# zju3dv/Diffuman4D

Hardware: NVIDIA H100
Metric: unet_window_denoise_steps_per_sec (higher is better)
Workload: dtype bf16

## Files before the change

diffuman4d_b200/csrc/common.cuh:

```cuda
#pragma once
#include <cuda.h>
#include <cuda_bf16.h>
#include <cuda_runtime.h>
#include <stdint.h>
#include <string>

namespace d4d {

typedef __nv_bfloat16 bf16;

void set_error(const std::string& msg);
#define D4D_CUDA_OK(expr)                                                                        \
  do {                                                                                           \
    cudaError_t _e = (expr);                                                                     \
    if (_e != cudaSuccess) {                                                                     \
      d4d::set_error(std::string(#expr) + " failed: " + cudaGetErrorString(_e) + " @" + __FILE__ + \
                     ":" + std::to_string(__LINE__));                                            \
      return 2;                                                                                  \
    }                                                                                            \
  } while (0)
#define D4D_REQUIRE(cond, msg)                                                                   \
  do {                                                                                           \
    if (!(cond)) {                                                                               \
      d4d::set_error(std::string("invalid argument: ") + msg + " (" #cond ") @" + __FILE__ + ":" + \
                     std::to_string(__LINE__));                                                  \
      return 1;                                                                                  \
    }                                                                                            \
  } while (0)

int make_tmap_2d(CUtensorMap* out, const void* base, uint64_t rows, uint64_t cols, uint64_t ld,
                 uint32_t box_cols, uint32_t box_rows, int swizzle_bytes);
int make_tmap_nhwc(CUtensorMap* out, const void* base, uint64_t n, uint64_t h, uint64_t w, uint64_t c,
                   uint32_t box_c, uint32_t box_w, uint32_t box_h, uint32_t box_n, int swizzle_bytes, int stride = 1);

#ifdef __CUDACC__
__device__ __forceinline__ uint32_t smem_u32(const void* p) {
  return static_cast<uint32_t>(__cvta_generic_to_shared(p));
}
__device__ __forceinline__ bool elect_one() {
  uint32_t pred = 0;
  asm volatile(
      "{\n\t.reg .b32 rx;\n\t.reg .pred px;\n\t"
      "elect.sync rx|px, 0xffffffff;\n\t"
      "selp.b32 %0, 1, 0, px;\n\t}\n"
      : "=r"(pred));
  return pred != 0;
}

__device__ __forceinline__ void mbar_init(uint64_t* bar, uint32_t count) {
  asm volatile("mbarrier.init.shared::cta.b64 [%0], %1;" ::"r"(smem_u32(bar)), "r"(count) : "memory");
}
__device__ __forceinline__ void fence_mbar_init() {
  asm volatile("fence.mbarrier_init.release.cluster;" ::: "memory");
}
__device__ __forceinline__ void mbar_expect_tx(uint64_t* bar, uint32_t bytes) {
  asm volatile("mbarrier.arrive.expect_tx.shared::cta.b64 _, [%0], %1;" ::"r"(smem_u32(bar)), "r"(bytes)
               : "memory");
}
__device__ __forceinline__ void mbar_arrive(uint64_t* bar) {
  asm volatile("mbarrier.arrive.shared::cta.b64 _, [%0];" ::"r"(smem_u32(bar)) : "memory");
}
__device__ __forceinline__ bool mbar_try_wait(uint64_t* bar, uint32_t parity) {
  uint32_t ok;
  asm volatile(
      "{\n\t.reg .pred p;\n\t"
      "mbarrier.try_wait.parity.shared::cta.b64 p, [%1], %2;\n\t"
      "selp.b32 %0, 1, 0, p;\n\t}\n"
      : "=r"(ok)
      : "r"(smem_u32(bar)), "r"(parity)
      : "memory");
  return ok != 0;
}
#ifndef D4D_SPIN_LIMIT
#define D4D_SPIN_LIMIT (1u << 26)
#endif
__device__ __forceinline__ void mbar_wait(uint64_t* bar, uint32_t parity) {
  uint32_t spins = 0;
  while (!mbar_try_wait(bar, parity)) {
    if (++spins > D4D_SPIN_LIMIT) {
      printf("d4d: mbarrier timeout block=(%d,%d) thread=%d bar=%u parity=%u\n", blockIdx.x, blockIdx.y,
             threadIdx.x, smem_u32(bar), parity);
      __trap();
    }
  }
}
__device__ __forceinline__ void mbar_wait_nocall(uint64_t* bar, uint32_t parity) {
  uint32_t spins = 0;
  while (!mbar_try_wait(bar, parity)) {
    if (++spins > D4D_SPIN_LIMIT) __trap();
  }
}

__device__ __forceinline__ void fence_proxy_async_smem() {
  asm volatile("fence.proxy.async.shared::cta;" ::: "memory");
}
__device__ __forceinline__ void named_barrier_sync(int id, int threads) {
  asm volatile("bar.sync %0, %1;" ::"r"(id), "r"(threads) : "memory");
}
__device__ __forceinline__ void named_barrier_arrive(int id, int threads) {
  asm volatile("bar.arrive %0, %1;" ::"r"(id), "r"(threads) : "memory");
}
__device__ __forceinline__ void st_shared_u32(uint32_t addr, uint32_t v) {
  asm volatile("st.shared.b32 [%0], %1;" ::"r"(addr), "r"(v) : "memory");
}
__device__ __forceinline__ uint32_t ld_shared_u32(uint32_t addr) {
  uint32_t v;
  asm volatile("ld.shared.b32 %0, [%1];" : "=r"(v) : "r"(addr) : "memory");
  return v;
}
__device__ __forceinline__ void pdl_wait() { asm volatile("griddepcontrol.wait;" ::: "memory"); }
__device__ __forceinline__ void pdl_launch_dependents() { asm volatile("griddepcontrol.launch_dependents;" ::: "memory"); }
template <int R> __device__ __forceinline__ void setmaxnreg_dec() { asm volatile("setmaxnreg.dec.sync.aligned.u32 %0;" ::"n"(R)); }
template <int R> __device__ __forceinline__ void setmaxnreg_inc() { asm volatile("setmaxnreg.inc.sync.aligned.u32 %0;" ::"n"(R)); }

__device__ __forceinline__ void tma_prefetch_desc(const CUtensorMap* t) {
  asm volatile("prefetch.tensormap [%0];" ::"l"(reinterpret_cast<uint64_t>(t)) : "memory");
}
__device__ __forceinline__ void tma_load_2d(void* dst, const CUtensorMap* t, uint64_t* bar, int c0, int c1) {
  asm volatile(
      "cp.async.bulk.tensor.2d.shared::cluster.global.tile.mbarrier::complete_tx::bytes [%0], [%1, {%3, %4}], [%2];"
      ::"r"(smem_u32(dst)), "l"(reinterpret_cast<uint64_t>(t)), "r"(smem_u32(bar)), "r"(c0), "r"(c1)
      : "memory");
}
__device__ __forceinline__ void tma_load_4d(void* dst, const CUtensorMap* t, uint64_t* bar, int c0, int c1, int c2,
                                            int c3) {
  asm volatile(
      "cp.async.bulk.tensor.4d.shared::cluster.global.tile.mbarrier::complete_tx::bytes [%0], [%1, {%3, %4, %5, %6}], [%2];"
      ::"r"(smem_u32(dst)), "l"(reinterpret_cast<uint64_t>(t)), "r"(smem_u32(bar)), "r"(c0), "r"(c1), "r"(c2),
      "r"(c3)
      : "memory");
}

__device__ __forceinline__ void tma_store_2d(const CUtensorMap* t, const void* src, int c0, int c1) {
  asm volatile("cp.async.bulk.tensor.2d.global.shared::cta.bulk_group [%0, {%2, %3}], [%1];"
               ::"l"(reinterpret_cast<uint64_t>(t)), "r"(smem_u32(src)), "r"(c0), "r"(c1) : "memory");
}
__device__ __forceinline__ void bulk_commit_group() { asm volatile("cp.async.bulk.commit_group;" ::: "memory"); }
template <int N> __device__ __forceinline__ void bulk_wait_group_read() {
  asm volatile("cp.async.bulk.wait_group.read %0;" ::"n"(N) : "memory");
}
template <int N> __device__ __forceinline__ void bulk_wait_group() {
  asm volatile("cp.async.bulk.wait_group %0;" ::"n"(N) : "memory");
}

__device__ __forceinline__ uint32_t pack_bf16x2(float lo, float hi) {
  __nv_bfloat162 v = __floats2bfloat162_rn(lo, hi);
  return *reinterpret_cast<uint32_t*>(&v);
}
__device__ __forceinline__ float2 unpack_bf16x2(uint32_t u) {
  __nv_bfloat162 v = *reinterpret_cast<__nv_bfloat162*>(&u);
  return __bfloat1622float2(v);
}
__device__ __forceinline__ float silu_f(float x) { return __fdividef(x, 1.0f + __expf(-x)); }
__device__ __forceinline__ float gelu_erf_f(float g) {
  const float u = fabsf(g);
  float q = fmaf(-4.8811754095e-04f, u, 7.1988063864e-03f);
  q = fmaf(q, u, -5.2146803588e-02f);
  q = fmaf(q, u, -4.5959571004e-01f);
  q = fmaf(q, u, -1.1510006189e+00f);
  float e;
  asm("ex2.approx.ftz.f32 %0, %1;" : "=f"(e) : "f"(q * u));
  return fmaf(-0.5f * u, e, fmaxf(g, 0.f));
}
#endif

}
```

diffuman4d_b200/csrc/gemm_wgmma.cu:

```cuda
#include "kernels.h"
#include "wgmma.cuh"

namespace d4d {

namespace {

constexpr int BLOCK_M = 128;
constexpr int BLOCK_K = 64;
constexpr int A_BYTES = BLOCK_M * BLOCK_K * 2;
constexpr int BAR_BYTES = 1024;
constexpr int NUM_THREADS = 384;
constexpr int MAX_SMEM = 227 * 1024;

constexpr int SLAB_COLS = 32;
constexpr int SLAB_BYTES = 64 * SLAB_COLS * 2;

template <int BN, int MI, bool kStaged, bool kPingPong>
struct GemmCfg {
  static constexpr int TILE_A_BYTES = kPingPong ? A_BYTES : MI * A_BYTES;
  static constexpr int STAGE_BYTES = TILE_A_BYTES + BN * BLOCK_K * 2;
  static constexpr int STAGING_BYTES = kStaged ? 2 * 64 * MI * BN * 2 : 0;
  static constexpr int STAGES_FIT = (MAX_SMEM - 1024 - BAR_BYTES - STAGING_BYTES) / STAGE_BYTES;
  static constexpr int STAGES = STAGES_FIT > 8 ? 8 : STAGES_FIT;
  static constexpr int SMEM = 1024 + BAR_BYTES + STAGES * STAGE_BYTES + STAGING_BYTES;
};

struct TileCoord {
  int m0;
  int n_img0, y0, x0;
  int pa, pb;
};

template <bool kConv>
__device__ __forceinline__ void tile_coords(const GemmKernelArgs& a, int m_tile, TileCoord& t) {
  if (!kConv) {
    t.m0 = m_tile * BLOCK_M;
    t.n_img0 = t.y0 = t.x0 = 0;
    t.pa = t.pb = 0;
  } else {
    const int ph = a.n_phases > 1 ? m_tile / a.tiles_per_phase : 0;
    m_tile -= ph * a.tiles_per_phase;
    t.pa = ph >> 1;
    t.pb = ph & 1;
    int tx = m_tile % a.tiles_x;
    int r = m_tile / a.tiles_x;
    int ty = r % a.tiles_y;
    int tn = r / a.tiles_y;
    t.m0 = 0;
    t.x0 = tx * a.BW;
    t.y0 = ty * a.BH;
    t.n_img0 = tn * a.BN;
  }
}

template <bool kConv>
__device__ __forceinline__ void row_of(const GemmKernelArgs& a, const TileCoord& tc, int rr, long long& row, int& img,
                                       bool& valid) {
  if (!kConv) {
    row = static_cast<long long>(tc.m0) + rr;
    valid = row < a.M;
    img = a.rows_per_image > 0 ? static_cast<int>(row / a.rows_per_image) : 0;
  } else {
    const int bx = rr % a.BW;
    const int r2 = rr / a.BW;
    const int by = r2 % a.BH;
    const int bn = r2 / a.BH;
    const int x = tc.x0 + bx, y = tc.y0 + by, n = tc.n_img0 + bn;
    valid = (x < a.W) && (y < a.H) && (n < a.n_img);
    row = (static_cast<long long>(n) * a.out_H + (y * a.out_sy + a.out_oy + tc.pa)) * a.out_W + (x * a.out_sx + a.out_ox + tc.pb);
    img = n;
  }
}

enum : int { E_BIAS = 1, E_ROWVEC = 2, E_ACT = 4, E_RES = 8, E_STATS = 16, E_KV = 32, E_ALL = 63, E_STAGED_ALL = E_ALL & ~E_KV };
__host__ __device__ constexpr bool gemm_staged(bool conv, int epi) { return !conv && !(epi & E_KV); }

constexpr int ORDER_BAR = 3;

template <int BN, int MI, bool kGeglu, bool kConv, int kEpi, bool kPingPong>
__global__ void __launch_bounds__(NUM_THREADS, 1)
gemm_wgmma_kernel(const __grid_constant__ CUtensorMap tmap_a, const __grid_constant__ CUtensorMap tmap_a2,
                  const __grid_constant__ CUtensorMap tmap_b, const __grid_constant__ CUtensorMap tmap_c,
                  const __grid_constant__ CUtensorMap tmap_r, const GemmKernelArgs a) {
  constexpr bool kStaged = gemm_staged(kConv, kEpi);
  static_assert(MI == 1 || (kConv && MI == 2) || kPingPong, "256-row tiles: conv mode only (a plain tile is 128 rows)");
  static_assert(!kPingPong || (kStaged && MI == 2), "ping-pong: staged plain GEMMs, one warpgroup per 128-row tile");
  using Cfg = GemmCfg<BN, MI, kStaged, kPingPong>;
  constexpr int STAGES = Cfg::STAGES;
  extern __shared__ uint8_t smem_raw[];
  uint8_t* smem = reinterpret_cast<uint8_t*>((reinterpret_cast<uintptr_t>(smem_raw) + 1023) & ~uintptr_t(1023));
  uint64_t* full = reinterpret_cast<uint64_t*>(smem);
  uint64_t* empty = full + STAGES;
  uint64_t* res_full = empty + STAGES;
  uint8_t* ring = smem + BAR_BYTES;

  const int warp = __shfl_sync(0xffffffffu, threadIdx.x >> 5, 0);
  const int lane = threadIdx.x & 31;
  const int total_tiles = a.m_tiles * a.n_tiles;

  if (threadIdx.x == 0) {
    tma_prefetch_desc(&tmap_a);
    tma_prefetch_desc(&tmap_b);
    if (a.kb_split < a.k_blocks) tma_prefetch_desc(&tmap_a2);
    for (int i = 0; i < STAGES; ++i) {
      mbar_init(&full[i], 1);
      mbar_init(&empty[i], kPingPong ? 1 : 2);
    }
    mbar_init(&res_full[0], 1);
    mbar_init(&res_full[1], 1);
    fence_mbar_init();
  }
  __syncthreads();
  pdl_wait();
  pdl_launch_dependents();

  if (warp < 4) {
    setmaxnreg_dec<40>();
    if (threadIdx.x == 0) {
      const uint32_t tx_bytes = Cfg::TILE_A_BYTES + static_cast<uint32_t>(a.block_n) * BLOCK_K * 2;
      int stage = 0;
      uint32_t phase = 0;
      for (int tile = blockIdx.x; tile < total_tiles; tile += gridDim.x) {
        const int m_tile = tile / a.n_tiles;
        const int n_tile = tile % a.n_tiles;
        TileCoord tc;
        tile_coords<kConv>(a, m_tile, tc);
        const int n0 = n_tile * a.block_n;
        for (int kb = 0; kb < a.k_blocks; ++kb) {
          mbar_wait_nocall(&empty[stage], phase ^ 1);
          uint8_t* sa = ring + stage * Cfg::STAGE_BYTES;
          uint8_t* sb = sa + Cfg::TILE_A_BYTES;
          mbar_expect_tx(&full[stage], tx_bytes);
          if (!kConv) {
            if (kb < a.kb_split) tma_load_2d(sa, &tmap_a, &full[stage], kb * BLOCK_K, tc.m0);
            else tma_load_2d(sa, &tmap_a2, &full[stage], (kb - a.kb_split) * BLOCK_K, tc.m0);
            tma_load_2d(sb, &tmap_b, &full[stage], kb * BLOCK_K, n0);
          } else {
            const int tap = kb / a.cin_blocks;
            const int cb = kb - tap * a.cin_blocks;
            tma_load_4d(sa, &tmap_a, &full[stage], cb * BLOCK_K, tc.x0 * a.in_stride + a.tap_dx[tap] + tc.pb,
                        tc.y0 * a.in_stride + a.tap_dy[tap] + tc.pa, tc.n_img0);
            tma_load_2d(sb, &tmap_b, &full[stage], tap * a.Cin + cb * BLOCK_K, n0 + (tc.pa * 2 + tc.pb) * a.N);
          }
          if (++stage == STAGES) { stage = 0; phase ^= 1; }
        }
      }
    }
    return;
  }

  setmaxnreg_inc<232>();
  const int wg = (warp >> 2) - 1;
  const int wq = warp & 3;
  const bool wg_leader = (threadIdx.x & 127) == 0;
  const int wg_row0 = kPingPong ? 0 : wg * 64 * MI;
  const int r_base = wg_row0 + wq * 16 + (lane >> 2);
  const int c_base = 2 * (lane & 3);
  const uint32_t ring_u32 = smem_u32(ring);
  constexpr int STG_BLOCK = 64 * BN * 2;
  const bool staged = kStaged && a.staged;
  uint8_t* stg = ring + STAGES * Cfg::STAGE_BYTES + wg * MI * STG_BLOCK;
  const uint32_t stg_u32 = smem_u32(stg) + (r_base - wg_row0) * 64 + c_base * 2;
  const int stg_xor = (lane >> 3) & 3;
  const bool has_res = (kEpi & E_RES) && !kGeglu && a.residual != nullptr;
  const int out_cols = kGeglu ? a.N / 2 : a.N;
  uint32_t res_phase = 0;

  int stage = 0;
  uint32_t phase = 0;
  const auto skip_stages = [&](int n) {
    stage += n;
    while (stage >= STAGES) { stage -= STAGES; phase ^= 1; }
  };
  if (kPingPong && wg == 1) {
    skip_stages(a.k_blocks);
    named_barrier_arrive(ORDER_BAR, 256);
  }
  const int tile_step = kPingPong ? 2 * gridDim.x : gridDim.x;
  float acc[MI][BN / 2];
  for (int tile = blockIdx.x + (kPingPong ? wg * gridDim.x : 0); tile < total_tiles; tile += tile_step) {
    const int m_tile = tile / a.n_tiles;
    const int n_tile = tile % a.n_tiles;
    TileCoord tc;
    tile_coords<kConv>(a, m_tile, tc);
    const int n0 = n_tile * a.block_n;
    const int ocol0 = kGeglu ? n0 / 2 : n0;
    const int ocols = min(kGeglu ? a.block_n / 2 : a.block_n, out_cols - ocol0);
    const int n_slabs = (ocols + SLAB_COLS - 1) / SLAB_COLS;
    const int orow0 = tc.m0 + wg_row0;
    const int live_blocks = staged ? max(0, min(MI, (a.M - orow0 + 63) / 64)) : 0;

    if (kPingPong) named_barrier_sync(ORDER_BAR + wg, 256);
    int prev_stage = -1;
    for (int kb = 0; kb < a.k_blocks; ++kb) {
      mbar_wait_nocall(&full[stage], phase);
      const uint32_t sa = ring_u32 + stage * Cfg::STAGE_BYTES + wg_row0 * 128;
      const uint32_t sb = ring_u32 + stage * Cfg::STAGE_BYTES + Cfg::TILE_A_BYTES;
      const uint64_t adesc = make_wgmma_desc(sa, 16, 1024);
      const uint64_t bdesc = make_wgmma_desc(sb, 16, 1024);
      wgmma_fence();
#pragma unroll
      for (int k = 0; k < BLOCK_K / 16; ++k) {
        const int scale_d = (kb | k) != 0 ? 1 : 0;
#pragma unroll
        for (int mi = 0; mi < MI; ++mi) {
          const uint64_t ad = adesc + 512 * mi + 2 * k, bd = bdesc + 2 * k;
          if constexpr (BN == 64) wgmma_ss_n64(acc[mi], ad, bd, scale_d);
          else if constexpr (BN == 128) wgmma_ss_n128(acc[mi], ad, bd, scale_d);
          else if constexpr (BN == 160) wgmma_ss_n160(acc[mi], ad, bd, scale_d);
          else if constexpr (BN == 192) wgmma_ss_n192(acc[mi], ad, bd, scale_d);
          else wgmma_ss_n256(acc[mi], ad, bd, scale_d);
        }
      }
      wgmma_commit();
      if (kb == 0 && staged && wg_leader) {
        bulk_wait_group_read<0>();
        if (has_res && live_blocks > 0) {
          mbar_expect_tx(&res_full[wg], live_blocks * n_slabs * SLAB_BYTES);
          for (int mi = 0; mi < live_blocks; ++mi)
            for (int s = 0; s < n_slabs; ++s)
              tma_load_2d(stg + mi * STG_BLOCK + s * SLAB_BYTES, &tmap_r, &res_full[wg], ocol0 + s * SLAB_COLS, orow0 + 64 * mi);
        }
      }
      wgmma_wait<1>();
      if (prev_stage >= 0 && wg_leader) mbar_arrive(&empty[prev_stage]);
      prev_stage = stage;
      if (++stage == STAGES) { stage = 0; phase ^= 1; }
    }
    if (kPingPong) {
      if (tile + gridDim.x < total_tiles) named_barrier_arrive(ORDER_BAR + (wg ^ 1), 256);
      skip_stages(a.k_blocks);
    }
    wgmma_wait<0>();
#pragma unroll
    for (int mi = 0; mi < MI; ++mi) wgmma_fence_regs(acc[mi]);
    if (wg_leader) mbar_arrive(&empty[prev_stage]);

    if (staged) {
      named_barrier_sync(1 + wg, 128);
      if (has_res && live_blocks > 0) {
        mbar_wait_nocall(&res_full[wg], res_phase);
        res_phase ^= 1;
      }
    }
#pragma unroll
    for (int mi = 0; mi < MI; ++mi) {
      auto stg_addr = [&](int j, int h) {
        return stg_u32 + mi * STG_BLOCK + h * 8 * 64 + (j >> 2) * SLAB_BYTES + (((j & 3) ^ stg_xor) << 4);
      };
      float (&accm)[BN / 2] = acc[mi];
      long long rows[2];
      int imgs[2];
      bool valid[2];
      row_of<kConv>(a, tc, r_base + 64 * mi, rows[0], imgs[0], valid[0]);
      row_of<kConv>(a, tc, r_base + 64 * mi + 8, rows[1], imgs[1], valid[1]);
      if constexpr (kGeglu) {
        const bool has_bias = (kEpi & E_BIAS) && a.bias != nullptr;
#pragma unroll
        for (int p = 0; p < BN / 16; ++p) {
          if (16 * p >= a.block_n || n0 + 16 * p >= a.N) break;
          float2 ba = make_float2(0.f, 0.f), bg = make_float2(0.f, 0.f);
          if (has_bias) {
            ba = __ldg(reinterpret_cast<const float2*>(a.bias + n0 + 16 * p + c_base));
            bg = __ldg(reinterpret_cast<const float2*>(a.bias + n0 + 16 * p + 8 + c_base));
          }
          const int ocol = n0 / 2 + 8 * p + c_base;
#pragma unroll
          for (int h = 0; h < 2; ++h) {
            if (!valid[h]) continue;
            const float a0 = accm[8 * p + 2 * h] + ba.x, a1 = accm[8 * p + 2 * h + 1] + ba.y;
            const float g0 = accm[8 * p + 4 + 2 * h] + bg.x, g1 = accm[8 * p + 4 + 2 * h + 1] + bg.y;
            const uint32_t o = pack_bf16x2(a0 * gelu_erf_f(g0), a1 * gelu_erf_f(g1));
            if (staged) st_shared_u32(stg_addr(p, h), o);
            else *reinterpret_cast<uint32_t*>(a.out + static_cast<size_t>(rows[h]) * a.ldo + ocol) = o;
          }
        }
      } else {
        const bool has_bias = (kEpi & E_BIAS) && a.bias != nullptr, has_rv = (kEpi & E_ROWVEC) && a.rowvec != nullptr;
        const bool has_stats = (kEpi & E_STATS) && a.stats != nullptr;
        const bool has_act = (kEpi & E_ACT) && a.act == 1, has_scale = (kEpi & E_ACT) && a.out_scale != 1.0f;
        const bool has_kv = (kEpi & E_KV) && a.kv_world > 0;
        const long long row0 = __shfl_sync(0xffffffffu, rows[0], 0);
        const bool stats_on = has_stats && __shfl_sync(0xffffffffu, valid[0] ? 1 : 0, 0);
        const int stats_img = !kConv ? static_cast<int>(row0 / a.stats_rows) : __shfl_sync(0xffffffffu, imgs[0], 0);
#pragma unroll
        for (int j = 0; j < BN / 8; ++j) {
          const int cl = 8 * j + c_base;
          const int col = n0 + cl;
          if (8 * j >= a.block_n || n0 + 8 * j >= a.N) break;
          float2 b2 = make_float2(0.f, 0.f);
          if (has_bias) b2 = __ldg(reinterpret_cast<const float2*>(a.bias + col));
          float sv[2][2];
#pragma unroll
          for (int h = 0; h < 2; ++h) {
            sv[h][0] = sv[h][1] = 0.f;
            if (!valid[h]) continue;
            float f0 = accm[4 * j + 2 * h] + b2.x, f1 = accm[4 * j + 2 * h + 1] + b2.y;
            if (has_rv) {
              const float2 v = unpack_bf16x2(*reinterpret_cast<const uint32_t*>(a.rowvec + static_cast<size_t>(imgs[h]) * a.ld_rowvec + col));
              f0 += v.x; f1 += v.y;
            }
            if (has_act) { f0 = silu_f(f0); f1 = silu_f(f1); }
            if (has_scale) { f0 *= a.out_scale; f1 *= a.out_scale; }
            if (has_res) {
              const float2 v = unpack_bf16x2(staged ? ld_shared_u32(stg_addr(j, h))
                                                    : *reinterpret_cast<const uint32_t*>(a.residual + static_cast<size_t>(rows[h]) * a.ld_res + col));
              f0 += v.x; f1 += v.y;
            }
            const uint32_t o = pack_bf16x2(f0, f1);
            if (has_stats) {
              const float2 rv = unpack_bf16x2(o);
              sv[h][0] = rv.x; sv[h][1] = rv.y;
            }
            if (has_kv && col >= a.kv_col0) {
              const long long half = rows[h] / a.kv_rows_local;
              const long long grow = half * a.kv_rows_global + a.kv_row_offset + (rows[h] - half * a.kv_rows_local);
              const size_t off = static_cast<size_t>(grow) * a.kv_ld + (col - a.kv_col0);
#pragma unroll 1
              for (int rk = 0; rk < a.kv_world; ++rk) *reinterpret_cast<uint32_t*>(a.kv_dst[rk] + off) = o;
            } else if (staged) {
              st_shared_u32(stg_addr(j, h), o);
            } else {
              *reinterpret_cast<uint32_t*>(a.out + static_cast<size_t>(rows[h]) * a.ldo + col) = o;
            }
          }
          if (has_stats) {
            float s0 = sv[0][0] + sv[1][0], s1 = sv[0][1] + sv[1][1];
            float q0 = sv[0][0] * sv[0][0] + sv[1][0] * sv[1][0], q1 = sv[0][1] * sv[0][1] + sv[1][1] * sv[1][1];
#pragma unroll
            for (int m = 4; m < 32; m <<= 1) {
              s0 += __shfl_xor_sync(0xffffffffu, s0, m);
              s1 += __shfl_xor_sync(0xffffffffu, s1, m);
              q0 += __shfl_xor_sync(0xffffffffu, q0, m);
              q1 += __shfl_xor_sync(0xffffffffu, q1, m);
            }
            if (stats_on && lane < 4) {
              unsigned long long* st = reinterpret_cast<unsigned long long*>(a.stats) + (static_cast<size_t>(stats_img) * a.N + col) * 2;
              atomicAdd(st + 0, static_cast<unsigned long long>(__float2ll_rn(s0 * kGnSumScale)));
              atomicAdd(st + 1, static_cast<unsigned long long>(__float2ll_rn(q0 * kGnSqScale)));
              atomicAdd(st + 2, static_cast<unsigned long long>(__float2ll_rn(s1 * kGnSumScale)));
              atomicAdd(st + 3, static_cast<unsigned long long>(__float2ll_rn(q1 * kGnSqScale)));
            }
          }
        }
      }
    }
    if (staged) {
      fence_proxy_async_smem();
      named_barrier_sync(1 + wg, 128);
      if (wg_leader && live_blocks > 0) {
        for (int mi = 0; mi < live_blocks; ++mi)
          for (int s = 0; s < n_slabs; ++s)
            tma_store_2d(&tmap_c, stg + mi * STG_BLOCK + s * SLAB_BYTES, ocol0 + s * SLAB_COLS, orow0 + 64 * mi);
        bulk_commit_group();
      }
    }
  }
  if (staged && wg_leader) bulk_wait_group<0>();
}

}

namespace {

void conv_out_grid(const GemmDesc& d, int* oh, int* ow, int* phases) {
  *oh = d.conv_kind == 1 ? d.H / 2 : d.H;
  *ow = d.conv_kind == 1 ? d.W / 2 : d.W;
  *phases = d.conv_kind == 3 ? 4 : 1;
}

struct ConvTile { int bw, bh, bn_img; long long tiles; };
ConvTile conv_tile(int rows, int n_img, int oh, int ow) {
  ConvTile t;
  t.bw = 16; while (t.bw > ow) t.bw >>= 1;
  t.bh = rows / t.bw; while (t.bh > oh && t.bh > 1) t.bh >>= 1;
  t.bn_img = rows / (t.bw * t.bh);
  t.tiles = static_cast<long long>((ow + t.bw - 1) / t.bw) * ((oh + t.bh - 1) / t.bh) * ((n_img + t.bn_img - 1) / t.bn_img);
  return t;
}

}

constexpr int kOperandWeight = 128;
constexpr int kMinKBlocks256 = 16;
constexpr int kEpilogueWeight = 3072;

namespace {
bool pingpong_width(int bn, bool geglu) { return bn == 128 || (bn == 64 && !geglu); }
}

int gemm_choose_tile(const GemmDesc& d, int sms, int* block_m, int* block_n, int* schedule) {
  D4D_REQUIRE(d.block_m == 0 || d.block_m == 128 || d.block_m == 256, "block_m must be 0 (automatic), 128 or 256");
  D4D_REQUIRE(d.block_m != 256 || d.conv, "256-row tiles: convolutions only (a plain GEMM stages a 128-row tile for its TMA store)");
  D4D_REQUIRE(d.block_m != 256 || d.block_n <= 0 || d.block_n == 128 || d.block_n == 160,
              "256-row tiles run at block_n 128 or 160 (the accumulators of wider tiles do not fit the register file)");
  D4D_REQUIRE(d.schedule == 0 || d.schedule == kSchedCooperative || d.schedule == kSchedPingPong,
              "schedule must be 0 (automatic), 1 (cooperative) or 2 (ping-pong)");
  const bool pp_ok = !d.conv && d.kv_world == 0;
  D4D_REQUIRE(d.schedule != kSchedPingPong || pp_ok, "ping-pong: plain GEMMs without the K/V scatter only");
  D4D_REQUIRE(d.schedule != kSchedPingPong || d.block_n <= 0 || pingpong_width(d.block_n, d.geglu),
              "ping-pong runs at block_n 64 or 128 (GEGLU: 128; wider accumulators do not fit the register file)");
  int oh = 0, ow = 0, phases = 1;
  if (d.conv) conv_out_grid(d, &oh, &ow, &phases);
  D4D_REQUIRE(!d.conv || (d.n_img > 0 && oh > 0 && ow > 0), "empty conv");
  const auto best_tile = [&](bool pingpong, int* bm, int* bn) {
    long long best_cost = -1;
    for (int r : {128, 256}) {
      if (d.block_m > 0 ? r != d.block_m : (r == 256 && !d.conv)) continue;
      if (pingpong && r != 128) continue;
      const int k_blocks = d.conv ? (d.conv_kind >= 2 ? 4 : 9) * ((d.Cin + BLOCK_K - 1) / BLOCK_K) : 0;
      const long long m_tiles = d.conv ? conv_tile(r, d.n_img, oh, ow).tiles * phases : (static_cast<long long>(d.M) + r - 1) / r;
// ... 53 lines not shown
}

int gemm_prepare(const GemmDesc& d, GemmLaunch* L) {
  D4D_REQUIRE(d.N % 16 == 0, "GEMM N must be a multiple of 16");
  D4D_REQUIRE(d.out != nullptr && d.A != nullptr && d.Wt != nullptr, "null operand");
  D4D_REQUIRE(d.kv_world >= 0 && d.kv_world <= 8, "K/V scatter: world must be in [1, 8]");
  if (d.kv_world > 0) {
    D4D_REQUIRE(!d.conv && !d.geglu && d.kv_col0 >= 0 && d.kv_col0 < d.N && d.kv_col0 % 16 == 0 && d.kv_ld % 8 == 0 &&
                d.kv_ld >= d.N - d.kv_col0, "K/V scatter arguments");
    for (int r = 0; r < d.kv_world; ++r) D4D_REQUIRE(d.kv_dst[r] != nullptr, "K/V scatter: null destination buffer");
    D4D_REQUIRE(d.kv_rows_local > 0 && d.M % d.kv_rows_local == 0, "K/V scatter: M must be a multiple of rows_local");
    D4D_REQUIRE(d.kv_row_offset >= 0 && d.kv_row_offset + d.kv_rows_local <= d.kv_rows_global,
                "K/V scatter: row_offset + rows_local exceeds rows_global");
  }
  GemmKernelArgs& a = L->args;
  memset(&a, 0, sizeof(a));
  int dev = 0, sms = 0;
  D4D_CUDA_OK(cudaGetDevice(&dev));
  D4D_CUDA_OK(cudaDeviceGetAttribute(&sms, cudaDevAttrMultiProcessorCount, dev));
  D4D_REQUIRE(d.block_n <= 0 || (d.block_n >= 16 && d.block_n <= 256 && d.block_n % 16 == 0 && d.N % d.block_n == 0),
              "no valid block_n");
  D4D_REQUIRE(!d.conv || (d.conv_kind >= 0 && d.conv_kind <= 3), "conv_kind");
  int bm = 0, bn = 0, sched = 0;
  if (int rc = gemm_choose_tile(d, sms, &bm, &bn, &sched)) return rc;
  a.block_m = bm;
  a.block_n = bn;
  a.n_tiles = (d.N + bn - 1) / bn;
  a.N = d.N;
  a.bias = d.bias;
  a.rowvec = d.rowvec;
  a.ld_rowvec = d.ld_rowvec;
  a.rows_per_image = d.rows_per_image;
  a.residual = d.residual;
  a.ld_res = d.ld_res;
  a.out = d.out;
  a.ldo = d.ldo;
  a.geglu = d.geglu;
  a.act = d.act;
  a.out_scale = d.out_scale;
  a.stats = d.stats;
  a.stats_rows = d.stats_rows > 0 ? d.stats_rows : 1;
  const char* no_stats = nullptr;
  D4D_REQUIRE(d.stats == nullptr || gemm_stats_fusable(d, sms, &no_stats), no_stats);
  a.kv_world = d.kv_world;
  a.kv_col0 = d.kv_col0;
  a.kv_ld = d.kv_ld;
  a.kv_rows_local = d.kv_rows_local > 0 ? d.kv_rows_local : 1;
  a.kv_rows_global = d.kv_rows_global;
  a.kv_row_offset = d.kv_row_offset;
  for (int i = 0; i < 8; ++i) a.kv_dst[i] = d.kv_dst[i];
  D4D_REQUIRE(d.ldo % 8 == 0 && (d.residual == nullptr || d.ld_res % 8 == 0) &&
              (d.rowvec == nullptr || d.ld_rowvec % 8 == 0), "leading dimensions must be multiples of 8");

  if (!d.conv) {
    D4D_REQUIRE(d.K1 > 0 && d.K1 % 8 == 0 && d.K2 % 8 == 0, "K must be a multiple of 8");
    D4D_REQUIRE(d.A2 == nullptr || d.K1 % BLOCK_K == 0, "two-source GEMM needs K1 % 64 == 0");
    a.mode = 0;
    a.M = d.M;
    a.m_tiles = (d.M + BLOCK_M - 1) / BLOCK_M;
    a.kb_split = (d.K1 + BLOCK_K - 1) / BLOCK_K;
    const int kb2 = d.A2 ? (d.K2 + BLOCK_K - 1) / BLOCK_K : 0;
    a.k_blocks = a.kb_split + kb2;
    const int K = d.K1 + (d.A2 ? d.K2 : 0);
    if (int rc = make_tmap_2d(&L->tmap_a, d.A, d.M, d.K1, d.lda, BLOCK_K, BLOCK_M, 128)) return rc;
    if (d.A2) {
      if (int rc = make_tmap_2d(&L->tmap_a2, d.A2, d.M, d.K2, d.lda2, BLOCK_K, BLOCK_M, 128)) return rc;
    } else {
      L->tmap_a2 = L->tmap_a;
    }
    if (int rc = make_tmap_2d(&L->tmap_b, d.Wt, d.N, K, K, BLOCK_K, bn, 128)) return rc;
    const auto aligned16 = [](const void* p) { return (reinterpret_cast<uintptr_t>(p) & 15) == 0; };
    a.staged = d.kv_world == 0 && (d.geglu ? bn % (2 * SLAB_COLS) : bn % SLAB_COLS) == 0 && aligned16(d.out) &&
               (d.residual == nullptr || aligned16(d.residual));
    D4D_REQUIRE(d.schedule != kSchedPingPong || a.staged, "ping-pong needs the staged epilogue (16-byte aligned out / residual)");
    a.pingpong = a.staged && sched == kSchedPingPong;
    L->tmap_c = L->tmap_r = L->tmap_a;
    if (a.staged) {
      if (int rc = make_tmap_2d(&L->tmap_c, d.out, d.M, d.geglu ? d.N / 2 : d.N, d.ldo, SLAB_COLS, 64, 64)) return rc;
      if (d.residual && !d.geglu)
        if (int rc = make_tmap_2d(&L->tmap_r, d.residual, d.M, d.N, d.ld_res, SLAB_COLS, 64, 64)) return rc;
    }
  } else {
    D4D_REQUIRE(d.Cin % 8 == 0, "conv Cin must be a multiple of 8");
    D4D_REQUIRE(d.conv_kind != 1 || (d.H % 2 == 0 && d.W % 2 == 0), "stride-2 conv needs even H, W");
    a.mode = 1;
    a.n_img = d.n_img; a.Cin = d.Cin;
    a.in_stride = 1; a.out_sy = a.out_sx = 1; a.out_oy = a.out_ox = 0;
    a.n_phases = 1;
    if (d.conv_kind >= 2) {
      const int pa = d.conv_kind == 3 ? 0 : d.up_a, pb = d.conv_kind == 3 ? 0 : d.up_b;
      a.n_taps = 4;
      for (int t = 0; t < 4; ++t) {
        a.tap_dy[t] = static_cast<signed char>((t >> 1) + pa - 1);
        a.tap_dx[t] = static_cast<signed char>((t & 1) + pb - 1);
      }
      a.H = d.H; a.W = d.W; a.out_H = 2 * d.H; a.out_W = 2 * d.W;
      a.out_sy = a.out_sx = 2; a.out_oy = pa; a.out_ox = pb;
      if (d.conv_kind == 3) a.n_phases = 4;
    } else {
      a.n_taps = 9;
      for (int t = 0; t < 9; ++t) {
        a.tap_dy[t] = static_cast<signed char>(t / 3 - 1);
        a.tap_dx[t] = static_cast<signed char>(t % 3 - 1);
      }
      if (d.conv_kind == 1) { a.in_stride = 2; a.H = d.H / 2; a.W = d.W / 2; }
      else { a.H = d.H; a.W = d.W; }
      a.out_H = a.H; a.out_W = a.W;
    }
    a.M = d.n_img * a.H * a.W;
    a.cin_blocks = (d.Cin + BLOCK_K - 1) / BLOCK_K;
    a.k_blocks = a.n_taps * a.cin_blocks;
    a.kb_split = a.k_blocks;
    const ConvTile ct = conv_tile(bm, d.n_img, a.H, a.W);
    const int bw = ct.bw, bh = ct.bh, bnimg = ct.bn_img;
    D4D_REQUIRE(bw * bh * bnimg == bm && bnimg <= 256, "conv tile shape");
    a.BW = bw; a.BH = bh; a.BN = bnimg;
    a.tiles_x = (a.W + bw - 1) / bw;
    a.tiles_y = (a.H + bh - 1) / bh;
    a.tiles_per_phase = static_cast<int>(ct.tiles);
    a.m_tiles = a.tiles_per_phase * a.n_phases;
    a.M *= a.n_phases;
    if (int rc = make_tmap_nhwc(&L->tmap_a, d.A, d.n_img, d.H, d.W, d.Cin, BLOCK_K, bw, bh, bnimg, 128, a.in_stride)) return rc;
    L->tmap_a2 = L->tmap_c = L->tmap_r = L->tmap_a;
    const uint64_t kw = static_cast<uint64_t>(a.n_taps) * d.Cin;
    if (int rc = make_tmap_2d(&L->tmap_b, d.Wt, static_cast<uint64_t>(d.N) * a.n_phases, kw, kw, BLOCK_K, bn, 128)) return rc;
  }
  const int total = a.m_tiles * a.n_tiles;
  L->grid = total < sms ? total : sms;
  return 0;
}

namespace {

using GemmKernelFn = void (*)(const CUtensorMap, const CUtensorMap, const CUtensorMap, const CUtensorMap,
                              const CUtensorMap, const GemmKernelArgs);
struct GemmVariant {
  int bn, bm;
  bool geglu, conv;
  int epi;
  bool pingpong;
  GemmKernelFn fn;
  int smem;
};
#define D4D_GV_M(BN, MI, G, C, E) \
  {BN, 128 * MI, G, C, E, false, gemm_wgmma_kernel<BN, MI, G, C, E, false>, GemmCfg<BN, MI, gemm_staged(C, E), false>::SMEM}
#define D4D_GV(BN, G, C, E) D4D_GV_M(BN, 1, G, C, E)
#define D4D_GV_PP(BN, G, E) \
  {BN, 128, G, false, E, true, gemm_wgmma_kernel<BN, 2, G, false, E, true>, GemmCfg<BN, 2, true, true>::SMEM}
#define D4D_GV_PLAIN(BN, GV)                                                                                          \
                                         \
  GV(BN, false, 0), GV(BN, false, E_BIAS), GV(BN, false, E_BIAS | E_RES), GV(BN, false, E_BIAS | E_RES | E_STATS),     \
  GV(BN, false, GV##_ALL)
#define D4D_GV_COOP_ALL E_ALL
#define D4D_GV_PP_ALL E_STAGED_ALL
#define D4D_GV_COOP(BN, G, E) D4D_GV(BN, G, false, E)
#define D4D_GV_CONV(BN, MI)                                                                                           \
                                                            \
  D4D_GV_M(BN, MI, false, true, E_BIAS | E_ROWVEC | E_STATS), D4D_GV_M(BN, MI, false, true, E_BIAS | E_RES | E_STATS), \
  D4D_GV_M(BN, MI, false, true, E_BIAS | E_STATS), D4D_GV_M(BN, MI, false, true, E_ALL)
const GemmVariant kGemmVariants[] = {
    D4D_GV_PLAIN(128, D4D_GV_COOP), D4D_GV_CONV(128, 1), D4D_GV_CONV(128, 2), D4D_GV(128, true, false, E_BIAS),
    D4D_GV_PLAIN(160, D4D_GV_COOP), D4D_GV_CONV(160, 1), D4D_GV_CONV(160, 2),
    D4D_GV_PLAIN(192, D4D_GV_COOP),
    D4D_GV_PLAIN(256, D4D_GV_COOP), D4D_GV_CONV(256, 1), D4D_GV(256, true, false, E_BIAS),
    D4D_GV(64, false, false, E_ALL), D4D_GV(64, false, true, E_ALL), D4D_GV(64, true, false, E_BIAS),
    D4D_GV_PLAIN(128, D4D_GV_PP), D4D_GV_PP(128, true, E_BIAS), D4D_GV_PP(64, false, E_STAGED_ALL),
};
#undef D4D_GV_COOP
#undef D4D_GV_COOP_ALL
#undef D4D_GV_PP_ALL
#undef D4D_GV_CONV
#undef D4D_GV_PLAIN
#undef D4D_GV_PP
#undef D4D_GV
#undef D4D_GV_M
constexpr int kNumGemmVariants = sizeof(kGemmVariants) / sizeof(kGemmVariants[0]);

int gemm_variant_at(const GemmKernelArgs& a, int bn) {
  const bool conv = a.mode != 0, geglu = a.geglu != 0;
  int need = 0;
  if (a.bias) need |= E_BIAS;
  if (!geglu) {
    if (a.rowvec) need |= E_ROWVEC;
    if (a.act == 1 || a.out_scale != 1.0f) need |= E_ACT;
    if (a.residual) need |= E_RES;
    if (a.stats) need |= E_STATS;
    if (a.kv_world > 0) need |= E_KV;
  }
  int generic = -1;
  for (int i = 0; i < kNumGemmVariants; ++i) {
    const GemmVariant& v = kGemmVariants[i];
    if (v.bn != bn || v.bm != a.block_m || v.geglu != geglu || v.conv != conv || v.pingpong != (a.pingpong != 0)) continue;
    if (v.epi == need) return i;
    if ((v.epi & need) == need && (generic < 0 || v.epi == E_ALL)) generic = i;
  }
  return generic;
}

// ... 29 lines not shown
```

diffuman4d_b200/csrc/tmap.cu:

```cuda
#include "common.cuh"

#include <mutex>

namespace d4d {

typedef CUresult (*EncodeTiledFn)(CUtensorMap*, CUtensorMapDataType, cuuint32_t, void*, const cuuint64_t*,
                                  const cuuint64_t*, const cuuint32_t*, const cuuint32_t*, CUtensorMapInterleave,
                                  CUtensorMapSwizzle, CUtensorMapL2promotion, CUtensorMapFloatOOBfill);

static EncodeTiledFn get_encode_fn() {
  static EncodeTiledFn fn = nullptr;
  static std::once_flag once;
  std::call_once(once, [] {
    void* p = nullptr;
    cudaDriverEntryPointQueryResult q;
    cudaError_t e = cudaGetDriverEntryPoint("cuTensorMapEncodeTiled", &p, cudaEnableDefault, &q);
    if (e == cudaSuccess && q == cudaDriverEntryPointSuccess) fn = reinterpret_cast<EncodeTiledFn>(p);
    else (void)cudaGetLastError();
  });
  return fn;
}

static CUtensorMapSwizzle swz(int bytes) {
  switch (bytes) {
// ... 5 lines not shown
}

int make_tmap_2d(CUtensorMap* out, const void* base, uint64_t rows, uint64_t cols, uint64_t ld, uint32_t box_cols,
                 uint32_t box_rows, int swizzle_bytes) {
  EncodeTiledFn fn = get_encode_fn();
  if (!fn) {
    set_error("cuTensorMapEncodeTiled unavailable (no CUDA driver?)");
    return 2;
  }
  D4D_REQUIRE((reinterpret_cast<uintptr_t>(base) & 15) == 0, "TMA base must be 16-byte aligned");
  D4D_REQUIRE((ld * 2) % 16 == 0, "TMA row pitch must be a multiple of 16 bytes");
  D4D_REQUIRE(box_cols <= 256 && box_rows <= 256 && box_cols >= 1 && box_rows >= 1, "TMA box dims must be in [1,256]");
  cuuint64_t gdim[2] = {cols, rows};
  cuuint64_t gstr[1] = {ld * 2};
  cuuint32_t box[2] = {box_cols, box_rows};
  cuuint32_t estr[2] = {1, 1};
  CUresult r = fn(out, CU_TENSOR_MAP_DATA_TYPE_BFLOAT16, 2, const_cast<void*>(base), gdim, gstr, box, estr,
                  CU_TENSOR_MAP_INTERLEAVE_NONE, swz(swizzle_bytes), CU_TENSOR_MAP_L2_PROMOTION_L2_256B,
                  CU_TENSOR_MAP_FLOAT_OOB_FILL_NONE);
  if (r != CUDA_SUCCESS) {
    set_error("cuTensorMapEncodeTiled(2d) failed, CUresult=" + std::to_string(static_cast<int>(r)) +
              " rows=" + std::to_string(rows) + " cols=" + std::to_string(cols) + " ld=" + std::to_string(ld) +
              " box=" + std::to_string(box_cols) + "x" + std::to_string(box_rows));
    return 2;
  }
  return 0;
}

int make_tmap_nhwc(CUtensorMap* out, const void* base, uint64_t n, uint64_t h, uint64_t w, uint64_t c, uint32_t box_c,
                   uint32_t box_w, uint32_t box_h, uint32_t box_n, int swizzle_bytes, int stride) {
  EncodeTiledFn fn = get_encode_fn();
  if (!fn) {
    set_error("cuTensorMapEncodeTiled unavailable (no CUDA driver?)");
    return 2;
  }
  D4D_REQUIRE((reinterpret_cast<uintptr_t>(base) & 15) == 0, "TMA base must be 16-byte aligned");
  D4D_REQUIRE((c * 2) % 16 == 0, "NHWC channel count must be a multiple of 8");
  cuuint64_t gdim[4] = {c, w, h, n};
  cuuint64_t gstr[3] = {c * 2, w * c * 2, h * w * c * 2};
  D4D_REQUIRE(stride >= 1 && stride <= 8 && box_w * stride <= 256 && box_h * stride <= 256, "TMA traversal stride");
  const cuuint32_t s = static_cast<cuuint32_t>(stride);
  cuuint32_t box[4] = {box_c, box_w * s, box_h * s, box_n};
  cuuint32_t estr[4] = {1, s, s, 1};
  CUresult r = fn(out, CU_TENSOR_MAP_DATA_TYPE_BFLOAT16, 4, const_cast<void*>(base), gdim, gstr, box, estr,
                  CU_TENSOR_MAP_INTERLEAVE_NONE, swz(swizzle_bytes), CU_TENSOR_MAP_L2_PROMOTION_L2_256B,
                  CU_TENSOR_MAP_FLOAT_OOB_FILL_NONE);
  if (r != CUDA_SUCCESS) {
    set_error("cuTensorMapEncodeTiled(4d) failed, CUresult=" + std::to_string(static_cast<int>(r)));
    return 2;
  }
  return 0;
}

}
```

Measured before the change: 14.47.

## Stage conv GEMM epilogues through shared memory with 5D TMA stores

Conv-mode implicit GEMMs now use the staged epilogue: output tiles are written to swizzled shared-memory slabs and stored with 5D TMA maps that cover both normal and 2x-upsampled NHWC outputs. Residuals are loaded the same way. Group-norm statistics are reduced per block in shared memory before one atomic per column, where shared memory allows, instead of many global atomics per warp. This is meant to cut uncoalesced direct global stores and atomic contention in conv epilogues. The costs are extra shared memory, which may reduce pipeline stages, and extra barriers per 64-row block.

```diff
diff --git a/diffuman4d_b200/csrc/common.cuh b/diffuman4d_b200/csrc/common.cuh
--- a/diffuman4d_b200/csrc/common.cuh
+++ b/diffuman4d_b200/csrc/common.cuh
@@ -32,6 +32,8 @@
                  uint32_t box_cols, uint32_t box_rows, int swizzle_bytes);
 int make_tmap_nhwc(CUtensorMap* out, const void* base, uint64_t n, uint64_t h, uint64_t w, uint64_t c,
                    uint32_t box_c, uint32_t box_w, uint32_t box_h, uint32_t box_n, int swizzle_bytes, int stride = 1);
+int make_tmap_5d(CUtensorMap* out, const void* base, const uint64_t dims[5], const uint64_t strides[4], const uint32_t box[5],
+                 int swizzle_bytes);
 
 #ifdef __CUDACC__
 __device__ __forceinline__ uint32_t smem_u32(const void* p) {
@@ -103,6 +105,14 @@
 __device__ __forceinline__ void st_shared_u32(uint32_t addr, uint32_t v) {
   asm volatile("st.shared.b32 [%0], %1;" ::"r"(addr), "r"(v) : "memory");
 }
+__device__ __forceinline__ void st_shared_u64(uint32_t addr, unsigned long long v) {
+  asm volatile("st.shared.b64 [%0], %1;" ::"r"(addr), "l"(v) : "memory");
+}
+__device__ __forceinline__ unsigned long long ld_shared_u64(uint32_t addr) {
+  unsigned long long v;
+  asm volatile("ld.shared.b64 %0, [%1];" : "=l"(v) : "r"(addr) : "memory");
+  return v;
+}
 __device__ __forceinline__ uint32_t ld_shared_u32(uint32_t addr) {
   uint32_t v;
   asm volatile("ld.shared.b32 %0, [%1];" : "=r"(v) : "r"(addr) : "memory");
@@ -135,6 +145,19 @@
   asm volatile("cp.async.bulk.tensor.2d.global.shared::cta.bulk_group [%0, {%2, %3}], [%1];"
                ::"l"(reinterpret_cast<uint64_t>(t)), "r"(smem_u32(src)), "r"(c0), "r"(c1) : "memory");
 }
+__device__ __forceinline__ void tma_load_5d(void* dst, const CUtensorMap* t, uint64_t* bar, int c0, int c1, int c2,
+                                            int c3, int c4) {
+  asm volatile(
+      "cp.async.bulk.tensor.5d.shared::cluster.global.tile.mbarrier::complete_tx::bytes [%0], [%1, {%3, %4, %5, %6, %7}], [%2];"
+      ::"r"(smem_u32(dst)), "l"(reinterpret_cast<uint64_t>(t)), "r"(smem_u32(bar)), "r"(c0), "r"(c1), "r"(c2),
+      "r"(c3), "r"(c4)
+      : "memory");
+}
+__device__ __forceinline__ void tma_store_5d(const CUtensorMap* t, const void* src, int c0, int c1, int c2, int c3, int c4) {
+  asm volatile("cp.async.bulk.tensor.5d.global.shared::cta.bulk_group [%0, {%2, %3, %4, %5, %6}], [%1];"
+               ::"l"(reinterpret_cast<uint64_t>(t)), "r"(smem_u32(src)), "r"(c0), "r"(c1), "r"(c2), "r"(c3), "r"(c4)
+               : "memory");
+}
 __device__ __forceinline__ void bulk_commit_group() { asm volatile("cp.async.bulk.commit_group;" ::: "memory"); }
 template <int N> __device__ __forceinline__ void bulk_wait_group_read() {
   asm volatile("cp.async.bulk.wait_group.read %0;" ::"n"(N) : "memory");
diff --git a/diffuman4d_b200/csrc/gemm_wgmma.cu b/diffuman4d_b200/csrc/gemm_wgmma.cu
--- a/diffuman4d_b200/csrc/gemm_wgmma.cu
+++ b/diffuman4d_b200/csrc/gemm_wgmma.cu
@@ -15,13 +15,20 @@
 constexpr int SLAB_COLS = 32;
 constexpr int SLAB_BYTES = 64 * SLAB_COLS * 2;
 
-template <int BN, int MI, bool kStaged, bool kPingPong>
+constexpr int ring_stages(int stage_bytes, int reserved) {
+  return (MAX_SMEM - 1024 - BAR_BYTES - reserved) / stage_bytes < 8 ? (MAX_SMEM - 1024 - BAR_BYTES - reserved) / stage_bytes : 8;
+}
+template <int BN, int MI, bool kStaged, bool kPingPong, bool kConv = false>
 struct GemmCfg {
   static constexpr int TILE_A_BYTES = kPingPong ? A_BYTES : MI * A_BYTES;
   static constexpr int STAGE_BYTES = TILE_A_BYTES + BN * BLOCK_K * 2;
-  static constexpr int STAGING_BYTES = kStaged ? 2 * 64 * MI * BN * 2 : 0;
-  static constexpr int STAGES_FIT = (MAX_SMEM - 1024 - BAR_BYTES - STAGING_BYTES) / STAGE_BYTES;
-  static constexpr int STAGES = STAGES_FIT > 8 ? 8 : STAGES_FIT;
+  static constexpr int STG_BLOCKS = kPingPong ? MI : 1;
+  static constexpr int SLABS_BYTES = kStaged ? 2 * 64 * STG_BLOCKS * BN * 2 : 0;
+  static constexpr int STATS_SLOTS_BYTES = 2 * 4 * BN * 2 * 8;
+  static constexpr bool BLOCK_STATS =
+      kStaged && kConv && ring_stages(STAGE_BYTES, SLABS_BYTES + STATS_SLOTS_BYTES) == ring_stages(STAGE_BYTES, SLABS_BYTES);
+  static constexpr int STAGING_BYTES = SLABS_BYTES + (BLOCK_STATS ? STATS_SLOTS_BYTES : 0);
+  static constexpr int STAGES = ring_stages(STAGE_BYTES, STAGING_BYTES);
   static constexpr int SMEM = 1024 + BAR_BYTES + STAGES * STAGE_BYTES + STAGING_BYTES;
 };
 
@@ -73,7 +80,39 @@
 }
 
 enum : int { E_BIAS = 1, E_ROWVEC = 2, E_ACT = 4, E_RES = 8, E_STATS = 16, E_KV = 32, E_ALL = 63, E_STAGED_ALL = E_ALL & ~E_KV };
-__host__ __device__ constexpr bool gemm_staged(bool conv, int epi) { return !conv && !(epi & E_KV); }
+__host__ __device__ constexpr bool gemm_staged(bool conv, int epi) { return conv || !(epi & E_KV); }
+
+template <bool kConv>
+__device__ __forceinline__ bool block_box(const GemmKernelArgs& a, const TileCoord& tc, int rr0, int (&c)[4]) {
+  if (!kConv) {
+    c[0] = c[1] = c[2] = 0;
+    c[3] = tc.m0 + rr0;
+    return c[3] < a.M;
+  }
+  const int r2 = rr0 / a.BW;
+  const int y = tc.y0 + r2 % a.BH, n = tc.n_img0 + r2 / a.BH;
+  c[1] = tc.x0;
+  if (a.out_sy == 2) {
+    c[0] = a.out_ox + tc.pb;
+    c[2] = a.out_oy + tc.pa;
+    c[3] = n * a.H + y;
+  } else {
+    c[0] = 0;
+    c[2] = y;
+    c[3] = n;
+  }
+  return y < a.H && n < a.n_img;
+}
+template <bool kConv>
+__device__ __forceinline__ void tma_load_slab(void* dst, const CUtensorMap* t, uint64_t* bar, int col, const int (&c)[4]) {
+  if (kConv) tma_load_5d(dst, t, bar, col, c[0], c[1], c[2], c[3]);
+  else tma_load_2d(dst, t, bar, col, c[3]);
+}
+template <bool kConv>
+__device__ __forceinline__ void tma_store_slab(const CUtensorMap* t, const void* src, int col, const int (&c)[4]) {
+  if (kConv) tma_store_5d(t, src, col, c[0], c[1], c[2], c[3]);
+  else tma_store_2d(t, src, col, c[3]);
+}
 
 constexpr int ORDER_BAR = 3;
 
@@ -85,7 +124,7 @@
   constexpr bool kStaged = gemm_staged(kConv, kEpi);
   static_assert(MI == 1 || (kConv && MI == 2) || kPingPong, "256-row tiles: conv mode only (a plain tile is 128 rows)");
   static_assert(!kPingPong || (kStaged && MI == 2), "ping-pong: staged plain GEMMs, one warpgroup per 128-row tile");
-  using Cfg = GemmCfg<BN, MI, kStaged, kPingPong>;
+  using Cfg = GemmCfg<BN, MI, kStaged, kPingPong, kConv>;
   constexpr int STAGES = Cfg::STAGES;
   extern __shared__ uint8_t smem_raw[];
   uint8_t* smem = reinterpret_cast<uint8_t*>((reinterpret_cast<uintptr_t>(smem_raw) + 1023) & ~uintptr_t(1023));
@@ -106,8 +145,8 @@
       mbar_init(&full[i], 1);
       mbar_init(&empty[i], kPingPong ? 1 : 2);
     }
-    mbar_init(&res_full[0], 1);
-    mbar_init(&res_full[1], 1);
+    mbar_init(&res_full[0], Cfg::STG_BLOCKS);
+    mbar_init(&res_full[1], Cfg::STG_BLOCKS);
     fence_mbar_init();
   }
   __syncthreads();
@@ -158,10 +197,13 @@
   const int c_base = 2 * (lane & 3);
   const uint32_t ring_u32 = smem_u32(ring);
   constexpr int STG_BLOCK = 64 * BN * 2;
+  constexpr int STG_BLOCKS = Cfg::STG_BLOCKS;
   const bool staged = kStaged && a.staged;
-  uint8_t* stg = ring + STAGES * Cfg::STAGE_BYTES + wg * MI * STG_BLOCK;
-  const uint32_t stg_u32 = smem_u32(stg) + (r_base - wg_row0) * 64 + c_base * 2;
-  const int stg_xor = (lane >> 3) & 3;
+  uint8_t* stg = ring + STAGES * Cfg::STAGE_BYTES + wg * STG_BLOCKS * STG_BLOCK;
+  const bool block_stats = Cfg::BLOCK_STATS && staged && (kEpi & E_STATS) && a.stats != nullptr;
+  const uint32_t sred = smem_u32(ring + STAGES * Cfg::STAGE_BYTES + 2 * STG_BLOCKS * STG_BLOCK) + wg * 4 * BN * 2 * 8;
+  if (block_stats)
+    for (int i = threadIdx.x & 127; i < 4 * BN * 2; i += 128) st_shared_u64(sred + i * 8, 0);
   const bool has_res = (kEpi & E_RES) && !kGeglu && a.residual != nullptr;
   const int out_cols = kGeglu ? a.N / 2 : a.N;
   uint32_t res_phase = 0;
@@ -187,8 +229,43 @@
     const int ocol0 = kGeglu ? n0 / 2 : n0;
     const int ocols = min(kGeglu ? a.block_n / 2 : a.block_n, out_cols - ocol0);
     const int n_slabs = (ocols + SLAB_COLS - 1) / SLAB_COLS;
-    const int orow0 = tc.m0 + wg_row0;
-    const int live_blocks = staged ? max(0, min(MI, (a.M - orow0 + 63) / 64)) : 0;
+    const auto load_residual = [&](int mi0) {
+      for (int i = 0; i < STG_BLOCKS; ++i) {
+        int c[4];
+        const bool live = block_box<kConv>(a, tc, wg_row0 + 64 * (mi0 + i), c);
+        mbar_expect_tx(&res_full[wg], live ? n_slabs * SLAB_BYTES : 0);
+        if (live)
+          for (int s = 0; s < n_slabs; ++s)
+            tma_load_slab<kConv>(stg + i * STG_BLOCK + s * SLAB_BYTES, &tmap_r, &res_full[wg], ocol0 + s * SLAB_COLS, c);
+      }
+    };
+    const auto store_blocks = [&](int mi0) {
+      fence_proxy_async_smem();
+      named_barrier_sync(1 + wg, 128);
+      if (wg_leader) {
+        for (int i = 0; i < STG_BLOCKS; ++i) {
+          int c[4];
+          if (block_box<kConv>(a, tc, wg_row0 + 64 * (mi0 + i), c))
+            for (int s = 0; s < n_slabs; ++s)
+              tma_store_slab<kConv>(&tmap_c, stg + i * STG_BLOCK + s * SLAB_BYTES, ocol0 + s * SLAB_COLS, c);
+        }
+        bulk_commit_group();
+      }
+      if (block_stats) {
+        const int r2 = (wg_row0 + 64 * mi0) / a.BW;
+        unsigned long long* st =
+            reinterpret_cast<unsigned long long*>(a.stats) + (static_cast<size_t>(tc.n_img0 + r2 / a.BH) * a.N + n0) * 2;
+        for (int i = threadIdx.x & 127; i < 2 * ocols; i += 128) {
+          unsigned long long v = 0;
+#pragma unroll
+          for (int w = 0; w < 4; ++w) {
+            v += ld_shared_u64(sred + (w * BN * 2 + i) * 8);
+            st_shared_u64(sred + (w * BN * 2 + i) * 8, 0);
+          }
+          if (v != 0) atomicAdd(st + i, v);
+        }
+      }
+    };
 
     if (kPingPong) named_barrier_sync(ORDER_BAR + wg, 256);
     int prev_stage = -1;
@@ -215,12 +292,7 @@
       wgmma_commit();
       if (kb == 0 && staged && wg_leader) {
         bulk_wait_group_read<0>();
-        if (has_res && live_blocks > 0) {
-          mbar_expect_tx(&res_full[wg], live_blocks * n_slabs * SLAB_BYTES);
-          for (int mi = 0; mi < live_blocks; ++mi)
-            for (int s = 0; s < n_slabs; ++s)
-              tma_load_2d(stg + mi * STG_BLOCK + s * SLAB_BYTES, &tmap_r, &res_full[wg], ocol0 + s * SLAB_COLS, orow0 + 64 * mi);
-        }
+        if (has_res) load_residual(0);
       }
       wgmma_wait<1>();
       if (prev_stage >= 0 && wg_leader) mbar_arrive(&empty[prev_stage]);
@@ -236,17 +308,25 @@
     for (int mi = 0; mi < MI; ++mi) wgmma_fence_regs(acc[mi]);
     if (wg_leader) mbar_arrive(&empty[prev_stage]);
 
-    if (staged) {
-      named_barrier_sync(1 + wg, 128);
-      if (has_res && live_blocks > 0) {
-        mbar_wait_nocall(&res_full[wg], res_phase);
-        res_phase ^= 1;
-      }
-    }
 #pragma unroll
     for (int mi = 0; mi < MI; ++mi) {
+      if (staged && mi % STG_BLOCKS == 0) {
+        if (mi > 0) {
+          store_blocks(mi - STG_BLOCKS);
+          if (wg_leader) {
+            bulk_wait_group_read<0>();
+            if (has_res) load_residual(mi);
+          }
+        }
+        named_barrier_sync(1 + wg, 128);
+        if (has_res) {
+          mbar_wait_nocall(&res_full[wg], res_phase);
+          res_phase ^= 1;
+        }
+      }
       auto stg_addr = [&](int j, int h) {
-        return stg_u32 + mi * STG_BLOCK + h * 8 * 64 + (j >> 2) * SLAB_BYTES + (((j & 3) ^ stg_xor) << 4);
+        return smem_u32(stg) + (mi % STG_BLOCKS) * STG_BLOCK + (r_base - wg_row0 + h * 8) * 64 + c_base * 2 +
+               (j >> 2) * SLAB_BYTES + (((j & 3) ^ ((lane >> 3) & 3)) << 4);
       };
       float (&accm)[BN / 2] = acc[mi];
       long long rows[2];
@@ -335,28 +415,28 @@
               q1 += __shfl_xor_sync(0xffffffffu, q1, m);
             }
             if (stats_on && lane < 4) {
-              unsigned long long* st = reinterpret_cast<unsigned long long*>(a.stats) + (static_cast<size_t>(stats_img) * a.N + col) * 2;
-              atomicAdd(st + 0, static_cast<unsigned long long>(__float2ll_rn(s0 * kGnSumScale)));
-              atomicAdd(st + 1, static_cast<unsigned long long>(__float2ll_rn(q0 * kGnSqScale)));
-              atomicAdd(st + 2, static_cast<unsigned long long>(__float2ll_rn(s1 * kGnSumScale)));
-              atomicAdd(st + 3, static_cast<unsigned long long>(__float2ll_rn(q1 * kGnSqScale)));
+              const unsigned long long v[4] = {static_cast<unsigned long long>(__float2ll_rn(s0 * kGnSumScale)),
+                                               static_cast<unsigned long long>(__float2ll_rn(q0 * kGnSqScale)),
+                                               static_cast<unsigned long long>(__float2ll_rn(s1 * kGnSumScale)),
+                                               static_cast<unsigned long long>(__float2ll_rn(q1 * kGnSqScale))};
+              if (block_stats) {
+#pragma unroll
+                for (int k = 0; k < 4; ++k) st_shared_u64(sred + ((wq * BN + cl) * 2 + k) * 8, v[k]);
+              } else {
+                unsigned long long* st = reinterpret_cast<unsigned long long*>(a.stats) + (static_cast<size_t>(stats_img) * a.N + col) * 2;
+#pragma unroll
+                for (int k = 0; k < 4; ++k) atomicAdd(st + k, v[k]);
+              }
             }
           }
         }
       }
     }
     if (staged) {
-      fence_proxy_async_smem();
-      named_barrier_sync(1 + wg, 128);
-      if (wg_leader && live_blocks > 0) {
-        for (int mi = 0; mi < live_blocks; ++mi)
-          for (int s = 0; s < n_slabs; ++s)
-            tma_store_2d(&tmap_c, stg + mi * STG_BLOCK + s * SLAB_BYTES, ocol0 + s * SLAB_COLS, orow0 + 64 * mi);
-        bulk_commit_group();
-      }
-    }
-  }
-  if (staged && wg_leader) bulk_wait_group<0>();
+      store_blocks(MI - STG_BLOCKS);
+      if (wg_leader && tile + tile_step >= total_tiles) bulk_wait_group<0>();
+    }
+  }
 }
 
 }
@@ -516,6 +596,7 @@
   D4D_REQUIRE(d.ldo % 8 == 0 && (d.residual == nullptr || d.ld_res % 8 == 0) &&
               (d.rowvec == nullptr || d.ld_rowvec % 8 == 0), "leading dimensions must be multiples of 8");
 
+  const auto aligned16 = [](const void* p) { return (reinterpret_cast<uintptr_t>(p) & 15) == 0; };
   if (!d.conv) {
     D4D_REQUIRE(d.K1 > 0 && d.K1 % 8 == 0 && d.K2 % 8 == 0, "K must be a multiple of 8");
     D4D_REQUIRE(d.A2 == nullptr || d.K1 % BLOCK_K == 0, "two-source GEMM needs K1 % 64 == 0");
@@ -533,7 +614,6 @@
       L->tmap_a2 = L->tmap_a;
     }
     if (int rc = make_tmap_2d(&L->tmap_b, d.Wt, d.N, K, K, BLOCK_K, bn, 128)) return rc;
-    const auto aligned16 = [](const void* p) { return (reinterpret_cast<uintptr_t>(p) & 15) == 0; };
     a.staged = d.kv_world == 0 && (d.geglu ? bn % (2 * SLAB_COLS) : bn % SLAB_COLS) == 0 && aligned16(d.out) &&
                (d.residual == nullptr || aligned16(d.residual));
     D4D_REQUIRE(d.schedule != kSchedPingPong || a.staged, "ping-pong needs the staged epilogue (16-byte aligned out / residual)");
@@ -588,6 +668,22 @@
     L->tmap_a2 = L->tmap_c = L->tmap_r = L->tmap_a;
     const uint64_t kw = static_cast<uint64_t>(a.n_taps) * d.Cin;
     if (int rc = make_tmap_2d(&L->tmap_b, d.Wt, static_cast<uint64_t>(d.N) * a.n_phases, kw, kw, BLOCK_K, bn, 128)) return rc;
+    a.staged = bn % SLAB_COLS == 0 && d.N >= SLAB_COLS && (bw * bh) % 64 == 0 && (a.out_sy == 1 || a.H % bh == 0) && aligned16(d.out) &&
+               (d.residual == nullptr || aligned16(d.residual));
+    if (a.staged) {
+      const auto out_map = [&](CUtensorMap* t, const bf16* base, int ld) {
+        const uint64_t w = a.W, px = static_cast<uint64_t>(ld);
+        const bool up = a.out_sy == 2;
+        const uint64_t dims[5] = {static_cast<uint64_t>(d.N), up ? 2u : 1u, w, up ? 2u : static_cast<uint64_t>(a.H),
+                                  up ? static_cast<uint64_t>(d.n_img) * a.H : static_cast<uint64_t>(d.n_img)};
+        const uint64_t strides[4] = {px, a.out_sx * px, a.out_W * px, a.out_W * px * (up ? 2 : a.H)};
+        const uint32_t box[5] = {SLAB_COLS, 1, static_cast<uint32_t>(bw), up ? 1u : 64u / bw, up ? 64u / bw : 1u};
+        return make_tmap_5d(t, base, dims, strides, box, 64);
+      };
+      if (int rc = out_map(&L->tmap_c, d.out, d.ldo)) return rc;
+      if (d.residual)
+        if (int rc = out_map(&L->tmap_r, d.residual, d.ld_res)) return rc;
+    }
   }
   const int total = a.m_tiles * a.n_tiles;
   L->grid = total < sms ? total : sms;
@@ -607,7 +703,7 @@
   int smem;
 };
 #define D4D_GV_M(BN, MI, G, C, E) \
-  {BN, 128 * MI, G, C, E, false, gemm_wgmma_kernel<BN, MI, G, C, E, false>, GemmCfg<BN, MI, gemm_staged(C, E), false>::SMEM}
+  {BN, 128 * MI, G, C, E, false, gemm_wgmma_kernel<BN, MI, G, C, E, false>, GemmCfg<BN, MI, gemm_staged(C, E), false, C>::SMEM}
 #define D4D_GV(BN, G, C, E) D4D_GV_M(BN, 1, G, C, E)
 #define D4D_GV_PP(BN, G, E) \
   {BN, 128, G, false, E, true, gemm_wgmma_kernel<BN, 2, G, false, E, true>, GemmCfg<BN, 2, true, true>::SMEM}
diff --git a/diffuman4d_b200/csrc/tmap.cu b/diffuman4d_b200/csrc/tmap.cu
--- a/diffuman4d_b200/csrc/tmap.cu
+++ b/diffuman4d_b200/csrc/tmap.cu
@@ -81,4 +81,33 @@
   return 0;
 }
 
+int make_tmap_5d(CUtensorMap* out, const void* base, const uint64_t dims[5], const uint64_t strides[4], const uint32_t box[5],
+                 int swizzle_bytes) {
+  EncodeTiledFn fn = get_encode_fn();
+  if (!fn) {
+    set_error("cuTensorMapEncodeTiled unavailable (no CUDA driver?)");
+    return 2;
+  }
+  D4D_REQUIRE((reinterpret_cast<uintptr_t>(base) & 15) == 0, "TMA base must be 16-byte aligned");
+  cuuint64_t gdim[5], gstr[4];
+  cuuint32_t bx[5], estr[5] = {1, 1, 1, 1, 1};
+  for (int i = 0; i < 5; ++i) {
+    D4D_REQUIRE(dims[i] >= 1 && box[i] >= 1 && box[i] <= 256, "TMA dims and box dims must be in [1, 256]");
+    gdim[i] = dims[i];
+    bx[i] = box[i];
+  }
+  for (int i = 0; i < 4; ++i) {
+    D4D_REQUIRE((strides[i] * 2) % 16 == 0, "TMA strides must be multiples of 16 bytes");
+    gstr[i] = strides[i] * 2;
+  }
+  CUresult r = fn(out, CU_TENSOR_MAP_DATA_TYPE_BFLOAT16, 5, const_cast<void*>(base), gdim, gstr, bx, estr,
+                  CU_TENSOR_MAP_INTERLEAVE_NONE, swz(swizzle_bytes), CU_TENSOR_MAP_L2_PROMOTION_L2_256B,
+                  CU_TENSOR_MAP_FLOAT_OOB_FILL_NONE);
+  if (r != CUDA_SUCCESS) {
+    set_error("cuTensorMapEncodeTiled(5d) failed, CUresult=" + std::to_string(static_cast<int>(r)));
+    return 2;
+  }
+  return 0;
 }
+
+}
```

Result: faster. 14.87 (median of 6 runs) (+2.8%).
